# radiocosmology/cora

Hardware: AMD Instinct MI355X
Metric: sky-maps/sec (nside=1024, lmax=2048, 256 freq) (higher is better)
Workload: dtype f64

## Files before the change

cora_amd/csrc/fft_shapes.h:

```cpp
#pragma once
#include <cstddef>
#include <type_traits>
#include <utility>

namespace fft_shapes {

struct ring_shape {
    int len;
    int nch;
    int mc;
    int t;
    int ana_t;
    bool own;
    double us;
};
inline constexpr ring_shape RING_DIRECT[] = {
    {2048, 4, 4, 512, 512, false, 9.9},
    {4096, 2, 8, 512, 512, false, 12.7},
};
inline constexpr ring_shape RING_BLU[] = {
    {8192, 1, 16, 256, 0, true, 26.1},
    {6144, 1, 8, 512, 0, true, 20.5},
    {4096, 2, 4, 512, 512, false, 15.0},
    {3584, 2, 4, 512, 512, true, 14.3},
    {3072, 2, 4, 512, 512, true, 13.3},
    {2560, 2, 4, 512, 512, true, 12.4},
    {2048, 4, 2, 512, 512, false, 12.6},
    {1536, 4, 2, 512, 512, true, 10.6},
    {1024, 4, 2, 256, 256, false, 6.8},
};
constexpr bool has_analysis(const ring_shape &s) { return s.ana_t != 0; }
constexpr bool own_filter(const ring_shape &s) { return s.own; }

struct line_shape {
    int len;
    int nch;
    int t = 512;
    int t_c2r = 512;
    bool h2 = false;
    int inner_min = 0;
};
inline constexpr line_shape LINE_REAL[] = {
    {256, 16, 512, 256}, {512, 16}, {1024, 8}, {2048, 4}, {192, 16, 512, 256}, {384, 16}, {768, 8}, {1536, 4},
};
inline constexpr line_shape LINE_C2C[] = {
    {256, 16, 256, 256, false, 16}, {512, 16, 512, 512, false, 16}, {1024, 16, 512, 512, true, 16},
    {1024, 8, 512, 512, false, 8},  {384, 16, 512, 512, false, 16}, {768, 8, 512, 512, false, 8},
};
inline constexpr line_shape LINE_BLU[] = {
    {256, 16},  {320, 16},  {384, 16},  {512, 16},  {640, 8},  {768, 8},  {1024, 8},
    {1280, 4},  {1536, 4},  {2048, 4},  {2560, 2},  {3072, 2}, {3584, 2}, {4096, 2},
};
constexpr int LINE_BLU_FILTER_T = 256;

template <size_t N>
constexpr bool whole_loads(const line_shape (&rows)[N]) {
    for (const line_shape &s : rows)
        if ((s.nch * s.len) % s.t != 0 || (s.nch * s.len) % s.t_c2r != 0) return false;
    return true;
}
static_assert(whole_loads(LINE_REAL) && whole_loads(LINE_C2C) && whole_loads(LINE_BLU), "(NCH * N) % T == 0");

template <class S, size_t N>
constexpr const S *find(const S (&rows)[N], int len) {
    for (const S &s : rows)
        if (s.len == len) return &s;
    return nullptr;
}
constexpr int ring_own_length(int h, int P) {
    int best = 0;
    for (const ring_shape &s : RING_BLU)
        if (s.own && s.len >= 2 * h - 1 && s.len <= P && (best == 0 || s.len < best)) best = s.len;
    return best;
}

template <const auto &ROWS, size_t I>
struct row_c {
    static constexpr auto row = ROWS[I];
};
template <auto KEEP, class S>
constexpr bool kept(const S &s) {
    if constexpr (std::is_null_pointer_v<decltype(KEEP)>) return true;
    else return KEEP(s);
}
template <const auto &ROWS, auto KEEP, size_t... I, class Match, class Launch>
int dispatch_rows(std::index_sequence<I...>, Match match, Launch launch, bool *took) {
    int rc = 0;
    auto one = [&](auto shape) {
        if constexpr (kept<KEEP>(shape.row)) {
            if (!match(shape.row)) return false;
            rc = launch(shape);
            *took = rc == 0;
            return true;
        } else {
            return false;
        }
    };
    (void)(one(row_c<ROWS, I>{}) || ...);
    return rc;
}
template <const auto &ROWS, auto KEEP = nullptr, class Match, class Launch>
int dispatch(Match match, Launch launch, bool *took) {
    *took = false;
    return dispatch_rows<ROWS, KEEP>(std::make_index_sequence<sizeof(ROWS) / sizeof(ROWS[0])>{}, match, launch, took);
}

template <template <int> class SCH, const auto &ROWS, size_t... I>
constexpr bool scheduled(std::index_sequence<I...>) {
    return ((SCH<ROWS[I].len>::R0 * SCH<ROWS[I].len>::R1 * SCH<ROWS[I].len>::R2 == ROWS[I].len) && ...);
}
template <template <int> class SCH, const auto &ROWS>
// ... 6 lines not shown
```

cora_amd/csrc/sht_internal.h:

```cpp
#pragma once
#include "common.h"

#include <algorithm>
#include <cmath>
#include <type_traits>
#include <cstdlib>
#include <map>

struct corahip_sht_plan {
    int nside = 0, lmax = 0, L = 0, npair = 0, nring = 0;
    int cut_exp = 0;
    std::map<int, uint64_t> k4_macro_steps;
    std::map<std::pair<int, int>, std::pair<int2 *, int>> k4_items;
    std::vector<int32_t> h_lmin;
    long npix = 0, nalm = 0;
    std::vector<int64_t> h_start;
    std::vector<int32_t> h_nphi;
    std::vector<double> h_z, h_sth, h_phi0;
    double *d_z = nullptr, *d_sth = nullptr;
    int32_t *d_nphi = nullptr;
    int64_t *d_start = nullptr;
    double *d_phi0 = nullptr;
    double2 *d_coef = nullptr;
    int32_t *d_lstart = nullptr;
// ... 375 lines not shown
                    zv.x *= invP;
                    zv.y *= invP;
                    *reinterpret_cast<double2 *>(out + 2 * jj) = zv;
                }
            }
        }
    }
}
#ifndef K5_MC_BLU4
#define K5_MC_BLU4 2
#endif
#define K5_MC 4
#ifndef K5_STAMPS
#define K5_STAMPS 0
#endif
#if K5_STAMPS
__device__ unsigned long long g_k5_stamps[8];
#define K5STAMP(acc) { unsigned long long _t; asm volatile("s_memtime %0\n\ts_waitcnt lgkmcnt(0)" : "=s"(_t)::"memory"); acc += _t - k5_last; k5_last = _t; }
#else
#define K5STAMP(acc)
#endif
static inline int nnu_pad_of(int nnu) { return (nnu + 7) & ~7; }
#define K5_TAIL_PAD ((size_t)8 * 512 * 64)

int sht_legendre(corahip_ctx *ctx, const corahip_sht_plan *p, int ncols, const double *alm, double *inter);
int sht_k4_items(corahip_ctx *ctx, const corahip_sht_plan *p, int rt, int ncg, const int2 **items, int *nitems);
int sht_k4_segseed(corahip_ctx *ctx, const corahip_sht_plan *p, int rt, const double2 **segseed);
int sht_legendre_pol(corahip_ctx *ctx, corahip_sht_plan *p, int ncols, const double *alm, double *inter);
int sht_ringfft(corahip_ctx *ctx, const corahip_sht_plan *p, const double *inter, int nnu_chunk_pad, int nnu_valid,
                double *maps);
int sht_ringfft_ct(corahip_ctx *ctx, const corahip_sht_plan *p, const corahip_sht_plan::ring_class &c, const double *inter,
                   int G, int nnu, double *maps, int cu_limit, bool *took);
bool sht_ringfft_ticketed(const corahip_sht_plan::ring_class &c);
double sht_ringfft_item_weight(const corahip_sht_plan::ring_class &c);
#define K5_NTICKETS 8
int sht_k5_tickets(corahip_ctx *ctx, hipStream_t stream);
int sht_ctfilt_tables(corahip_ctx *ctx, corahip_sht_plan *p);
int sht_second_stream(corahip_ctx *ctx);
struct StreamRestore {
    corahip_ctx *c;
    hipStream_t s;
    bool forked = false;
    int fork() {
        const int rc = sht_second_stream(c);
        if (rc) return rc;
        HIP_TRY(hipEventRecord(c->ev_fork, s));
        HIP_TRY(hipStreamWaitEvent(c->stream2, c->ev_fork, 0));
        forked = true;
        return 0;
    }
    int join() {
        c->stream = s;
        HIP_TRY(hipEventRecord(c->ev_join, c->stream2));
        HIP_TRY(hipStreamWaitEvent(s, c->ev_join, 0));
        forked = false;
        return 0;
    }
    ~StreamRestore() {
        c->stream = s;
        if (forked && (hipEventRecord(c->ev_join, c->stream2) != hipSuccess || hipStreamWaitEvent(s, c->ev_join, 0) != hipSuccess))
            (void)hipStreamSynchronize(c->stream2);
    }
};
int sht_ringana_ct(corahip_ctx *ctx, const corahip_sht_plan *p, const corahip_sht_plan::ring_class &c, const double *maps, int nvalid,
                   int nnu_pad, const double *ring_w, int G, double *inter, bool *took);
int sht_ringana(corahip_ctx *ctx, const corahip_sht_plan *p, const double *maps, int nnu, int nnu_pad8,
                const double *ring_w, double *inter);
int sht_legendre_adj(corahip_ctx *ctx, const corahip_sht_plan *p, int ncols, const double *inter, double *part,
// ... 2 lines not shown
```

cora_amd/csrc/sht_ringfft.hip:

```cpp
#include "sht_internal.h"

template <int NCH, bool BLU>
__global__ void __launch_bounds__(K5_THREADS)
ringfft_kernel(const int32_t *__restrict__ ring_list, int nlist, int nside, int lmax, int G, int nnu, long npix,
               const int32_t *__restrict__ nphi_a, const int64_t *__restrict__ start_a,
               const double *__restrict__ phi0_a, const double *__restrict__ inter, double *__restrict__ maps,
               const double2 *__restrict__ tw_hbm, int pmax, const int32_t *__restrict__ blu_P,
               const int64_t *__restrict__ boff, const int64_t *__restrict__ foff,
               const double2 *__restrict__ chirp, const double2 *__restrict__ filt, int bstride,
               const int32_t *__restrict__ mcut) {
    constexpr int MC = BLU ? (NCH == 4 ? K5_MC_BLU4 : (K5_MC > 2 ? 2 : K5_MC)) : K5_MC;
    extern __shared__ __attribute__((aligned(16))) double2 sm[];
    const int tid = threadIdx.x, nt = blockDim.x;
    const int L = lmax + 1;
    const int ngrp = (nnu + NCH - 1) / NCH;
    const int nitems = nlist * ngrp;
    double *smd = reinterpret_cast<double *>(sm);
    const double2 *tw = tw_hbm;

    struct cell_t {
        double re[NCH], im[NCH];
    };
    cell_t pf0, pf1, pf2, pf3;
    auto cell_ptr = [&](int item) {
// ... 370 lines not shown
                *reinterpret_cast<double2 *>(cell + 4) = make_double2(im[0], im[1 % NCH]);
            } else {
                cell[0] = re[0];
                cell[4] = im[0];
            }
        }
    }
}
namespace {
struct ClassTimer {
    bool on;
    hipStream_t stream;
    hipEvent_t e0 = nullptr, e1 = nullptr;
    ClassTimer(bool on_, hipStream_t stream_) : on(on_), stream(stream_) {
        if (!on) return;
        (void)hipEventCreate(&e0);
        (void)hipEventCreate(&e1);
        (void)hipEventRecord(e0, stream);
    }
    void report(const char *kernel, const corahip_sht_plan::ring_class &c, int cus) {
        if (!on) return;
        float ms = 0.f;
        (void)hipEventRecord(e1, stream);
        (void)hipEventSynchronize(e1);
        (void)hipEventElapsedTime(&ms, e0, e1);
        fprintf(stderr, "%s class P=%d (length %d) nch=%d rings=%d: %.3f ms on %d CUs\n", kernel, c.blu ? c.len : 0, c.length(), c.nch,
                c.count, ms, cus);
        (void)hipEventDestroy(e0);
        (void)hipEventDestroy(e1);
    }
};
}

static int ringfft_launch_class(corahip_ctx *ctx, const corahip_sht_plan *p, const corahip_sht_plan::ring_class &c,
                                const double *inter, int G, int nnu_valid, double *maps, int cu_limit) {
    bool took = false;
    const int rct = sht_ringfft_ct(ctx, p, c, inter, G, nnu_valid, maps, cu_limit, &took);
    if (rct) return rct;
    if (took) return 0;
    const size_t shm = sizeof(double2) * (size_t)c.nch * c.bstride;
    const long nitems = (long)c.count * ((nnu_valid + c.nch - 1) / c.nch);
    const int per_cu = std::max<int>(1, (int)((160 * 1024) / std::max<size_t>(shm, 1)));
    const int k5_threads = c.threads ? c.threads : K5_THREADS;
    dim3 grid((unsigned)std::min<long>(nitems, (long)cu_limit * std::min(per_cu, k5_threads <= 128 ? 8 : 4)));
#define RINGFFT_LAUNCH(NCH, BLU)                                                                                     \
    HIP_TRY(hipFuncSetAttribute((const void *)ringfft_kernel<NCH, BLU>, hipFuncAttributeMaxDynamicSharedMemorySize,  \
                                160 * 1024));                                                                   \
    ringfft_kernel<NCH, BLU><<<grid, k5_threads, shm, ctx->stream>>>(c.d_list, c.count, p->nside, p->lmax, G, nnu_valid, p->npix,     \
                                                         p->d_nphi, p->d_start, p->d_phi0, inter, maps, p->d_tw, \
                                                         p->pmax, p->d_blu_P, p->d_blu_boff, p->d_blu_foff,      \
                                                         p->d_bchirp, p->d_bfilt, c.bstride, p->d_mcut)
    if (!c.blu) {
        if (c.nch == 4) { RINGFFT_LAUNCH(4, false); }
        else if (c.nch == 2) { RINGFFT_LAUNCH(2, false); }
        else { RINGFFT_LAUNCH(1, false); }
    } else {
        if (c.nch == 4) { RINGFFT_LAUNCH(4, true); }
        else if (c.nch == 2) { RINGFFT_LAUNCH(2, true); }
        else { RINGFFT_LAUNCH(1, true); }
    }
#undef RINGFFT_LAUNCH
    LAUNCH_CHECK();
    return 0;
}

static int k5_belt_wgs_switch() {
    const char *e = getenv("CORAHIP_K5_BELT_WGS");
    if (!e || !*e) return -1;
    return std::max(0, atoi(e));
}

int sht_ringfft(corahip_ctx *ctx, const corahip_sht_plan *p, const double *inter, int nnu_chunk_pad, int nnu_valid,
                       double *maps) {
    {
        StageTimer t(ctx, "ringfft");
        const int G = nnu_chunk_pad / 4;
        static const bool class_times = getenv("CORAHIP_K5_TIMES") != nullptr;
        const bool two = !class_times && !K5_STAMPS && p->classes.size() > 1;
        hipStream_t const main_stream = ctx->stream;
        StreamRestore restore{ctx, main_stream};
        const int ncu = ctx->num_cu;

        const corahip_sht_plan::ring_class *belt = nullptr;
        std::vector<std::pair<double, const corahip_sht_plan::ring_class *>> side;
        double B = 0.0, C = 0.0;
        for (const auto &c : p->classes) {
            const double cost = 1e-3 * sht_ringfft_item_weight(c) * (double)c.count * ((nnu_valid + c.nch - 1) / c.nch);
            if (!belt && sht_ringfft_ticketed(c)) {
                belt = &c;
                B = cost;
            } else {
                side.push_back({cost, &c});
                C += cost;
            }
        }
        if (belt) {
            const int rct = sht_k5_tickets(ctx, main_stream);
            if (rct) return rct;
        }
        const int sw = k5_belt_wgs_switch();
        int W = 0;
        if (two && belt && !side.empty() && sw != 0 && ncu >= 16 && ncu % 8 == 0) {
            if (sw > 0) {
                W = std::min(std::max(8 * ((sw + 4) / 8), 8), ncu - 8);
            } else if (B >= 0.2 * ncu && C >= 0.2 * ncu) {
                int gran = 8;
                for (const auto &sc : side) gran = std::max(gran, sc.second->nch == 2 ? 16 : (sc.second->nch == 1 ? 32 : 8));
                if (ncu % gran) gran = 8;
                const double share = C / (B + C) * ncu;
                int S = gran * (int)std::ceil(share / gran + 0.1);
                S = std::min(std::max(S, gran), ncu - 8);
                W = ncu - S;
            }
        }
        if (W > 0) {
            int rc = restore.fork();
            if (rc) return rc;
            if ((rc = ringfft_launch_class(ctx, p, *belt, inter, G, nnu_valid, maps, W))) return rc;
            ctx->stream = ctx->stream2;
            std::stable_sort(side.begin(), side.end(), [](const auto &a, const auto &b) { return a.first > b.first; });
            for (const auto &sc : side)
                if ((rc = ringfft_launch_class(ctx, p, *sc.second, inter, G, nnu_valid, maps, ncu - W))) return rc;
            if ((rc = ringfft_launch_class(ctx, p, *belt, inter, G, nnu_valid, maps, ncu - W))) return rc;
            return restore.join();
        }

        int rc = two ? restore.fork() : 0;
        if (rc) return rc;
        int launch_no = 0;
        for (const auto &c : p->classes) {
            if (two) ctx->stream = (launch_no++ & 1) ? ctx->stream2 : main_stream;
            ClassTimer timer(class_times, ctx->stream);
            const int cus = (class_times && sw > 0 && &c == belt) ? std::min(sw, ncu) : ncu;
            if ((rc = ringfft_launch_class(ctx, p, c, inter, G, nnu_valid, maps, cus))) return rc;
            timer.report("K5", c, cus);
#if K5_STAMPS
            {
                unsigned long long hs[8];
                HIP_TRY(hipStreamSynchronize(ctx->stream));
                HIP_TRY(hipMemcpyFromSymbol(hs, HIP_SYMBOL(g_k5_stamps), sizeof(hs)));
                fprintf(stderr, "K5 class P=%d nch=%d rings=%d: pre %llu zero %llu fold %llu z %llu fft %llu out %llu mid %llu dit %llu\n",
                        c.blu ? c.len : 0, c.nch, c.count, hs[0], hs[1], hs[2], hs[3], hs[4], hs[5], hs[6], hs[7]);
                unsigned long long z8[8] = {0};
                HIP_TRY(hipMemcpyToSymbol(HIP_SYMBOL(g_k5_stamps), z8, sizeof(z8)));
            }
#endif
        }
        if (two) return restore.join();
    }
    return 0;
}

int sht_ringana(corahip_ctx *ctx, const corahip_sht_plan *p, const double *maps, int nnu, int nnu_pad8,
                const double *ring_w, double *inter) {
    StageTimer t(ctx, "ringana");
    const int G = nnu_pad8 / 4;
// ... 35 lines not shown
```

cora_amd/csrc/sht_ringfft_ct.hip:

```cpp
#include "sht_internal.h"

#define CT_T 512
#ifndef CT_STAMPS
#define CT_STAMPS 0
#endif
#if CT_STAMPS
__device__ unsigned long long g_ct_stamps[12];
#define CTSTAMP(k) { unsigned long long _t; asm volatile("s_memtime %0\n\ts_waitcnt lgkmcnt(0)" : "=s"(_t)::"memory"); ct_acc[k] += _t - ct_last; ct_last = _t; }
#else
#define CTSTAMP(k)
#endif

#include "fft_ct.h"
#include "fft_shapes.h"
static_assert(fft_shapes::scheduled<Sch, fft_shapes::RING_DIRECT>() && fft_shapes::scheduled<Sch, fft_shapes::RING_BLU>(),
              "every ring shape has its three-pass schedule");

template <int NCH>
struct cell_ct {
    double re[NCH], im[NCH];
};
template <int NCH>
__device__ __forceinline__ static cell_ct<NCH> load_cell_ct(const double *cell, unsigned m) {
    cell_ct<NCH> c;
// ... 102 lines not shown
#pragma unroll
        for (int k = 0; k < MC; k++) {
            if (tid + k * T < Lr) fold_cell<PK, NCH, BS>(sm, tid + k * T, n, h, noalias, ph, pf[k]);
            ph = cmul(ph, phstep);
        }
        if (TAIL) {
            if (tid + MC * T < Lr) fold_cell<PK, NCH, BS>(sm, tid + MC * T, n, h, noalias, ph, pf[MC]);
            ph = cmul(ph, phstep);
        }
        for (int m = tid + (MC + (TAIL ? 1 : 0)) * T; m < Lr; m += T) {
            fold_cell<PK, NCH, BS>(sm, m, n, h, noalias, ph, load_cell_ct<NCH>(cell, m));
            ph = cmul(ph, phstep);
        }
    }
};

template <int NCH>
__device__ __forceinline__ static int ct_remap(int v, int nitems) {
    constexpr int SH = NCH == 2 ? 1 : (NCH == 1 ? 2 : 0);
    const bool on = SH > 0 && (nitems & ((8 << SH) - 1)) == 0 && (gridDim.x & ((8 << SH) - 1)) == 0;
    if (!on) return v;
    const int slot = v >> 3, xcd = v & 7;
    return (((slot >> SH) * 8 + xcd) << SH) + (slot & ((1 << SH) - 1));
}

template <int NCH>
__device__ __forceinline__ static int ct_remap_tk(int v, int nitems) {
    constexpr int SH = NCH == 2 ? 1 : (NCH == 1 ? 2 : 0);
    if (SH == 0 || (nitems & ((8 << SH) - 1)) != 0) return v;
    const int slot = v >> 3, xcd = v & 7;
    return (((slot >> SH) * 8 + xcd) << SH) + (slot & ((1 << SH) - 1));
}

template <int N, int NCH, int MC, int T>
__global__ void __launch_bounds__(T)
ringfft_direct_ct(const int32_t *__restrict__ ring_list, int nlist, int lmax, int G, int nnu, long npix,
                  const int64_t *__restrict__ start_a, const double *__restrict__ phi0_a,
                  const double *inter, double *maps, const int32_t *__restrict__ mcut, int *tickets) {
    constexpr int PK = K5_PK_DIRECT;
    constexpr int R0 = Sch<N>::R0, R1 = Sch<N>::R1, R2 = Sch<N>::R2;
    static_assert(R0 == 16 && R1 == 16, "digit map of the fused store assumes 16 x 16 x R2");
    constexpr int Q0 = N / R0;
    static_assert(Q0 % 128 == 0, "first-pass stride must be a multiple of the padding period");
    constexpr int BS = fpc(N) + 1 + K5_CH_SKEW;
    constexpr int n = 2 * N, h = N;
    extern __shared__ __attribute__((aligned(16))) double2 sm[];
    const int tid0 = threadIdx.x;
    const int L = lmax + 1;
    const int ngrp = (nnu + NCH - 1) / NCH;
    const int nitems = nlist * ngrp;

    constexpr bool PERX = NCH < 4;
    __shared__ int s_tk[2];
    int *ctr = tickets + (PERX ? (int)(blockIdx.x & 7) : 0);
    auto vitem_of = [&](int t) { return PERX ? 8 * t + (int)(blockIdx.x & 7) : t; };
    int tkn = 0;

    double2 wH, wA, wB;
    hermitian_twiddles<N, Q0, R1>(tid0, wH, wA, wB);
    auto cell_ptr = [&](int item) {
        const int ring = ring_list[item / ngrp];
        const int ch0 = (item % ngrp) * NCH;
        return inter + ((size_t)ring * G + (ch0 >> 2)) * L * 8 + (ch0 & 3);
    };
    FrontEnd<PK, NCH, BS, MC, true, T> fe;
    double2 phS, phstepS;
// ... 81 lines not shown
            constexpr int TOT = NCH * 256;
            constexpr int IT = (TOT + T - 1) / T;
            fe.touch();
            if (tid0 == 0) s_tk[1] = tkn;
#pragma unroll
            for (int it = 0; it < IT; it++) {
                const int idx = tid + it * T;
                if ((TOT % T) != 0 && idx >= TOT) break;
                const int ch = idx >> 8;
                int k0, k1;
                fused_digits<R0>(idx & 255, k0, k1);
                const double2 *p = sm + ch * BS + fused_slot<PK, R2>(k0, k1);
                double2 x[R2];
#pragma unroll
                for (int r = 0; r < R2; r++) x[r] = p[fpc(r)];
                DftR<R2, 1>::run(x);
                if (ch0 + ch < nnu) {
                    double *out = maps + (size_t)(ch0 + ch) * npix + start + 2 * (k0 + 16 * k1);
#pragma unroll
                    for (int r = 0; r < R2; r++) *reinterpret_cast<double2 *>(out + 512 * r) = x[r];
                }
            }
        }
        vitem = vnext;
    }
}

template <int P, int NCH, int MC, int T>
__global__ void __launch_bounds__(T)
ringfft_blu_ct(const int32_t *__restrict__ ring_list, int nlist, int nside, int lmax, int G, int nnu, long npix,
               const int32_t *__restrict__ nphi_a, const int64_t *__restrict__ start_a,
               const double *__restrict__ phi0_a, const double *inter, double *maps,
               const int64_t *__restrict__ boff, const int64_t *__restrict__ foff, const double2 *chirp,
               const double2 *filt, const int32_t *__restrict__ mcut, const double2 *foldph, const double2 *foldstep) {
    constexpr int PK = K5_PK_BLU;
    constexpr int R0 = Sch<P>::R0, R1 = Sch<P>::R1, R2 = Sch<P>::R2;
    constexpr int Q0 = P / R0;
    constexpr int BS = fpc(P) + K5_CH_SKEW;
    constexpr int HALF = (R0 / 2) * Q0;
    constexpr int U = (HALF / 2 + ((P & (P - 1)) ? 1 : 0) + T - 1) / T;
    extern __shared__ __attribute__((aligned(16))) double2 sm[];
    const int tid0 = threadIdx.x;
    const int L = lmax + 1;
    const int ngrp = (nnu + NCH - 1) / NCH;
    const int nitems = nlist * ngrp;
    const double invP = 1.0 / (double)P;

    double2 wA, wB;
    pass_twiddles<P, Q0, R1>(tid0, wA, wB);
    auto cell_ptr = [&](int item) {
        const int ring = ring_list[item / ngrp];
        const int ch0 = (item % ngrp) * NCH;
        return inter + ((size_t)ring * G + (ch0 >> 2)) * L * 8 + (ch0 & 3);
    };
    FrontEnd<PK, NCH, BS, MC, false, T, (U > 4 ? U : 4)> fe;
    double2 cbn[U];
    auto load_cbn = [&](int item, int t) {
        const int ring = ring_list[item / ngrp];
        const int ic = ring + 1 < nside ? ring + 1 : 4 * nside - (ring + 1);
        const double2 *b = chirp + boff[ic - 1];
        const int hh = nphi_a[ring] >> 1;
#pragma unroll
        for (int u = 0; u < U; u++) cbn[u] = b[min(t + u * T, hh - 1)];
    };
    int vitem = blockIdx.x;
    if (vitem < nitems) {
        fe.prefetch(cell_ptr(ct_remap<NCH>(vitem, nitems)), L, tid0);
        load_cbn(ct_remap<NCH>(vitem, nitems), tid0);
    }
    fe.touch();
#pragma unroll
    for (int u = 0; u < U; u++) asm volatile("" ::"v"(cbn[u].x), "v"(cbn[u].y));
#if CT_STAMPS
    unsigned long long ct_acc[12] = {0, 0, 0, 0, 0, 0, 0, 0, 0, 0, 0, 0}, ct_last;
    { unsigned long long _t; asm volatile("s_memtime %0\n\ts_waitcnt lgkmcnt(0)" : "=s"(_t)::"memory"); ct_last = _t; }
#endif
    for (; vitem < nitems; vitem += gridDim.x) {
        int tid = tid0;
        asm volatile("" : "+v"(tid));
        const int item = ct_remap<NCH>(vitem, nitems);
        const int ring = ring_list[item / ngrp];
        const int ch0 = (item % ngrp) * NCH;
        const int n = nphi_a[ring];
        const int h = n >> 1;
        const long start = start_a[ring];
        const int icap = ring + 1 < nside ? ring + 1 : 4 * nside - (ring + 1);
        const int Lr = mcut[ring];
        const double2 *bch = chirp + boff[icap - 1];
        constexpr int BPT = (P / R2 + T - 1) / T;
        const double2 *f = filt + foff[icap - 1] + (size_t)(tid % (P / R2)) * R2;
        constexpr bool FL_EARLY = !(R0 > 16 && T == 512);
        double2 fl[BPT][R2];
        if constexpr (FL_EARLY)
#pragma unroll
        for (int q = 0; q < BPT; q++)
#pragma unroll
            for (int r = 0; r < (R2 + 1) / 2; r++) fl[q][r] = f[(size_t)min(q * T, P / R2 - 1 - (int)(tid % (P / R2))) * R2 + r];
        const double2 fph0 = foldph[(size_t)(icap - 1) * 512 + tid];
        const double2 fphs = foldstep[(icap - 1) * 2 + (T == 512 ? 1 : 0)];
        double2 cb[U];
#pragma unroll
        for (int u = 0; u < U; u++) cb[u] = cbn[u];
        __syncthreads();
        CTSTAMP(0);
        fe.fold(sm, cell_ptr(item), Lr, n, fph0, fphs, tid);
        CTSTAMP(1);
        if constexpr (FL_EARLY)
#pragma unroll
        for (int q = 0; q < BPT; q++)
#pragma unroll
            for (int r = (R2 + 1) / 2; r < R2; r++) fl[q][r] = f[(size_t)min(q * T, P / R2 - 1 - (int)(tid % (P / R2))) * R2 + r];
        __syncthreads();
        CTSTAMP(2);
        static_assert(U <= decltype(fe)::KP, "the pre-pass takes w^k from the fold phases that are kept");
#pragma unroll
        for (int u = 0; u < U; u++) {
            const int k = tid + u * T;
            if (2 * k <= h) {
                const int k2 = h - k;
                const double2 wk = csqr(fe.phk[u]);
                const double2 iw = make_double2(-wk.y, wk.x);
                const double2 miwc = make_double2(-wk.y, -wk.x);
#pragma unroll
                for (int c = 0; c < NCH; c++) {
                    double2 *bc = sm + c * BS;
                    const double2 xa = bc[fpad(k)], xb = bc[fpad(k2)];
                    const double2 s1 = make_double2(xa.x + xb.x, xa.y - xb.y), d1 = make_double2(xa.x - xb.x, xa.y + xb.y);
                    const double2 s2 = make_double2(s1.x, -s1.y), d2 = make_double2(-d1.x, d1.y);
                    const double2 zk = cmul(cb[u], cadd(s1, cmul(iw, d1)));
                    const double2 zk2 = cmul(cb[u], cadd(s2, cmul(miwc, d2)));
                    bc[fpad(k)] = zk;
                    if (k > 0) {
                        if (k2 != k) bc[fpad(k2)] = zk2;
                    } else {
                        bc[fpad(h)] = make_double2(0.0, 0.0);
                    }
                }
            }
        }
        for (int j = h + 1 + tid; j < HALF; j += T)
#pragma unroll
            for (int c = 0; c < NCH; c++) sm[c * BS + fpad(j)] = make_double2(0.0, 0.0);
        const int nitem = ct_remap<NCH>(min(vitem + (int)gridDim.x, nitems - 1), nitems);
        fe.template prefetch<0>(cell_ptr(nitem), L, tid);
        __syncthreads();
        CTSTAMP(3);
        {
            constexpr int TOT = NCH * Q0;
            constexpr int IT = (TOT + T - 1) / T;
            const double2 w = cconj(wA);
#pragma unroll
            for (int it = 0; it < IT; it++) {
                const int idx = tid + it * T;
                if ((TOT % T) != 0 && idx >= TOT) break;
                const int ch = idx / Q0, j0 = idx & (Q0 - 1);
                double2 *p = sm + ch * BS + fpad(j0);
                double2 x[R0];
#pragma unroll
                for (int r = 0; r < R0 / 2; r++) x[r] = p[fpc(r * Q0)];
#pragma unroll
                for (int r = R0 / 2; r < R0; r++) x[r] = make_double2(0.0, 0.0);
                DftR<R0, -1>::run(x);
                tw_apply<R0>(x, w);
#pragma unroll
                for (int r = 0; r < R0; r++) p[fpc(r * Q0)] = x[r];
            }
        }
        fe.template prefetch<1>(cell_ptr(nitem), L, tid);
        load_cbn(nitem, tid);
        if constexpr (!FL_EARLY) {
#pragma unroll
            for (int r = 0; r < R2; r++) fl[0][r] = f[r];
        }
        __syncthreads();
        CTSTAMP(4);
        ct_pass<PK, P, NCH, BS, Q0, R1, -1, false, T>(sm, wB, tid);
// ... 14 lines not shown
                    for (int r = 0; r < R2; r++) x[r] = p[fpc(r)];
                    DftR<R2, -1>::run(x);
#pragma unroll
                    for (int r = 0; r < R2; r++) x[r] = cmul(x[r], fl[0][r]);
                    DftR<R2, 1>::run(x);
#pragma unroll
                    for (int r = 0; r < R2; r++) p[fpc(r)] = x[r];
                }
            } else {
#pragma unroll
                for (int ch = 0; ch < NCH; ch++)
#pragma unroll
                    for (int q = 0; q < BPT; q++) {
                        if ((NB % T) != 0 && tid + q * T >= NB) break;
                        double2 *p = sm + ch * BS + fpad((tid + q * T) * R2);
                        double2 x[R2];
#pragma unroll
                        for (int r = 0; r < R2; r++) x[r] = p[fpc(r)];
                        DftR<R2, -1>::run(x);
#pragma unroll
                        for (int r = 0; r < R2; r++) x[r] = cmul(x[r], fl[q][r]);
                        DftR<R2, 1>::run(x);
#pragma unroll
                        for (int r = 0; r < R2; r++) p[fpc(r)] = x[r];
                    }
            }
        }
        constexpr bool OB_EARLY = R0 <= 16;
        double2 ob[R0 / 2];
        if constexpr (OB_EARLY) blu_out_chirps<P>(ob, bch, tid & (Q0 - 1), h);
        __syncthreads();
        CTSTAMP(6);
        ct_pass<PK, P, NCH, BS, Q0, R1, 1, true, T>(sm, wB, tid);
        __syncthreads();
        CTSTAMP(7);
        {
            constexpr int TOT = NCH * Q0;
            constexpr int IT = (TOT + T - 1) / T;
#pragma unroll
            for (int it = 0; it < IT; it++) {
                const int idx = tid + it * T;
                if ((TOT % T) != 0 && idx >= TOT) break;
                const int ch = idx / Q0, j0 = idx & (Q0 - 1);
                const double2 *p = sm + ch * BS + fpad(j0);
                double2 x[R0];
#pragma unroll
                for (int r = 0; r < R0; r++) x[r] = p[fpc(r * Q0)];
                tw_apply<R0>(x, wA);
                DftR<R0, 1>::run(x);
                if (ch0 + ch < nnu) {
                    double *out = maps + (size_t)(ch0 + ch) * npix + start;
#pragma unroll
                    for (int r = 0; r < R0 / 2; r++) {
                        const int jj = j0 + r * Q0;
                        if (jj < h) {
                            double2 zv = cmul(x[r], OB_EARLY ? ob[r] : bch[jj]);
                            zv.x *= invP;
                            zv.y *= invP;
                            *reinterpret_cast<double2 *>(out + 2 * jj) = zv;
                        }
                    }
                }
            }
        }
        CTSTAMP(8);
    }
#if CT_STAMPS
    if ((tid0 & 63) == 0)
        for (int k = 0; k < 9; k++) atomicAdd(&g_ct_stamps[k], ct_acc[k]);
#endif
}

template <int N, int NCH, int T>
__global__ void __launch_bounds__(T)
ringana_direct_ct(const int32_t *__restrict__ ring_list, int nlist, int lmax, int G, int nnu, int nvalid, long npix,
                  const int64_t *__restrict__ start_a, const double *__restrict__ phi0_a, const double *maps, double *inter,
                  const int32_t *__restrict__ mcut, const double *__restrict__ ring_w, int nring) {
    constexpr int PK = K5_PK_DIRECT;
    constexpr int R0 = Sch<N>::R0, R1 = Sch<N>::R1, R2 = Sch<N>::R2;
    static_assert(R0 == 16 && R1 == 16, "digit map of the fused load assumes 16 x 16 x R2");
    constexpr int Q0 = N / R0;
    static_assert(Q0 % 128 == 0, "first-pass stride must be a multiple of the padding period");
    constexpr int BS = fpc(N) + 1 + K5_CH_SKEW;
    constexpr int TOT0 = NCH * 256, IT0 = (TOT0 + T - 1) / T;
    static_assert(TOT0 % T == 0, "every thread loads whole butterflies");
    constexpr int MO = N / T;
    extern __shared__ __attribute__((aligned(16))) double2 sm[];
    const int tid0 = threadIdx.x;
    const int L = lmax + 1;
    const int ngrp = (nnu + NCH - 1) / NCH;
    const int nitems = nlist * ngrp;

    double2 wA, wB;
    double2 wS, wSstep;
    double2 phS, phSstep;
    pass_twiddles<N, Q0, R1>(tid0, wA, wB);
    {
        double s, c;
// ... 74 lines not shown
#pragma unroll
            for (int u = 0; u < MO; u++) {
                const int m = tid + u * T;
                if (m < Lr) emit(m, w, ph);
                w = cmul(w, wSstep);
                ph = cmul(ph, phstep);
            }
            if (tid == 0 && N < Lr) emit(N, make_double2(-1.0, 0.0), shifted ? make_double2(0.0, -1.0) : make_double2(1.0, 0.0));
        }
    }
}

template <int N, int NCH, int MC, int T>
static int launch_direct(corahip_ctx *ctx, hipStream_t stream, const corahip_sht_plan *p,
                         const corahip_sht_plan::ring_class &c, const double *inter, int G, int nnu, double *maps, int cu_limit) {
    constexpr int PK = K5_PK_DIRECT;
    constexpr int BS = fpc(N) + 1 + K5_CH_SKEW;
    const long nitems = (long)c.count * ((nnu + NCH - 1) / NCH);
    const auto [shm, grid] = ct_launch_geom(NCH, BS, 0, 0, nitems, cu_limit);
    if (!ctx->k5_tickets) {
        corahip_set_error("ring FFT: the ticket counters of the context are missing");
        return CORAHIP_ESTATE;
    }
    static_assert(sizeof(double2) * (size_t)NCH * BS + 64 <= 160 * 1024, "channel buffers + ticket words fit the LDS");
    HIP_TRY(hipFuncSetAttribute((const void *)ringfft_direct_ct<N, NCH, MC, T>, hipFuncAttributeMaxDynamicSharedMemorySize,
                                (int)shm));
    ringfft_direct_ct<N, NCH, MC, T><<<grid, T, shm, stream>>>(c.d_list, c.count, p->lmax, G, nnu, p->npix, p->d_start,
                                                               p->d_phi0, inter, maps, p->d_mcut, ctx->k5_tickets);
    LAUNCH_CHECK();
    return 0;
}
template <int P, int NCH, int MC, int T>
static int launch_blu(corahip_ctx *ctx, hipStream_t stream, const corahip_sht_plan *p,
                      const corahip_sht_plan::ring_class &c, const double *inter, int G, int nnu, double *maps, int cu_limit) {
    const int64_t *d_foff = c.ct_own ? p->d_ctfilt_off : p->d_blu_foff;
    const double2 *d_filt = c.ct_own ? p->d_ctfilt : p->d_bfilt;
    constexpr int PK = K5_PK_BLU;
    constexpr int BS = fpc(P) + K5_CH_SKEW;
    static_assert(sizeof(double2) * (size_t)NCH * BS <= 160 * 1024, "channel buffers fit the LDS");
    const long nitems = (long)c.count * ((nnu + NCH - 1) / NCH);
    const auto [shm, grid] = ct_launch_geom(NCH, BS, 0, 0, nitems, cu_limit);
    HIP_TRY(hipFuncSetAttribute((const void *)ringfft_blu_ct<P, NCH, MC, T>, hipFuncAttributeMaxDynamicSharedMemorySize,
                                160 * 1024));
    ringfft_blu_ct<P, NCH, MC, T><<<grid, T, shm, stream>>>(c.d_list, c.count, p->nside, p->lmax, G, nnu, p->npix, p->d_nphi,
                                                            p->d_start, p->d_phi0, inter, maps, p->d_blu_boff,
                                                            d_foff, p->d_bchirp, d_filt, p->d_mcut, p->d_foldph, p->d_foldstep);
    LAUNCH_CHECK();
#if CT_STAMPS
    {
        unsigned long long hs[12], z[12] = {0};
        HIP_TRY(hipStreamSynchronize(stream));
        HIP_TRY(hipMemcpyFromSymbol(hs, HIP_SYMBOL(g_ct_stamps), sizeof(hs)));
        const double per = 1.0 / ((double)nitems * (T / 64));
        fprintf(stderr, "K5ct P=%d nch=%d items=%ld: cycles/item  top %.0f fold %.0f pf+bar %.0f pre %.0f F1 %.0f F2 %.0f mid %.0f I2 %.0f I3 %.0f\n",
                P, NCH, nitems, hs[0] * per, hs[1] * per, hs[2] * per, hs[3] * per, hs[4] * per, hs[5] * per, hs[6] * per,
                hs[7] * per, hs[8] * per);
        HIP_TRY(hipMemcpyToSymbol(HIP_SYMBOL(g_ct_stamps), z, sizeof(z)));
    }
#endif
    return 0;
}

int sht_ringfft_ct(corahip_ctx *ctx, const corahip_sht_plan *p, const corahip_sht_plan::ring_class &c, const double *inter,
                   int G, int nnu, double *maps, int cu_limit, bool *took) {
    const auto len_is = [&](const fft_shapes::ring_shape &s) { return s.len == c.ct_len; };
    if (!c.blu)
        return fft_shapes::dispatch<fft_shapes::RING_DIRECT>(len_is, [&](auto shape) {
            return launch_direct<shape.row.len, shape.row.nch, shape.row.mc, shape.row.t>(ctx, ctx->stream, p, c, inter, G, nnu, maps, cu_limit);
        }, took);
    return fft_shapes::dispatch<fft_shapes::RING_BLU>(len_is, [&](auto shape) {
        return launch_blu<shape.row.len, shape.row.nch, shape.row.mc, shape.row.t>(ctx, ctx->stream, p, c, inter, G, nnu, maps, cu_limit);
    }, took);
}

template <int P, int NCH, int T>
__global__ void __launch_bounds__(T)
ringana_blu_ct(const int32_t *__restrict__ ring_list, int nlist, int nside, int lmax, int G, int nnu, int nvalid, long npix,
               const int32_t *__restrict__ nphi_a, const int64_t *__restrict__ start_a, const double *maps, double *inter,
               const int64_t *__restrict__ boff, const int64_t *__restrict__ foff, const double2 *chirp, const double2 *filt,
               const int32_t *__restrict__ mcut, const double2 *foldph, const double2 *foldstep, const double *__restrict__ ring_w) {
    constexpr int PK = K5_PK_BLU;
    constexpr int R0 = Sch<P>::R0, R1 = Sch<P>::R1, R2 = Sch<P>::R2;
    static_assert(R0 <= 16, "the lengths above 4096 keep the generic kernel");
    constexpr int Q0 = P / R0;
    constexpr int BS = fpc(P) + K5_CH_SKEW;
    constexpr int HALF = (R0 / 2) * Q0;
    constexpr int U = (HALF + T - 1) / T;
    constexpr int NB = P / R2;
    static_assert(NB <= T, "one middle-stage butterfly per thread and channel group");
    extern __shared__ __attribute__((aligned(16))) double2 sm[];
    const int tid0 = threadIdx.x;
    const int L = lmax + 1;
    const int ngrp = (nnu + NCH - 1) / NCH;
    const int nitems = nlist * ngrp;
    const int nring = 4 * nside - 1;
    const double invP = 1.0 / (double)P;

    double2 wA, wB;
    pass_twiddles<P, Q0, R1>(tid0, wA, wB);
    double2 pf[NCH][U];
    double2 cbn[U];
    auto prefetch = [&](int item, int t) {
        const int ring = ring_list[item / ngrp];
        const int ch0 = (item % ngrp) * NCH;
// ... 163 lines not shown
}
template <int P, int NCH, int T>
static int launch_ana_blu(corahip_ctx *ctx, hipStream_t stream, const corahip_sht_plan *p, const corahip_sht_plan::ring_class &c,
                          const double *maps, int nvalid, int nnu_pad, const double *ring_w, int G, double *inter) {
    constexpr int PK = K5_PK_BLU;
    constexpr int BS = fpc(P) + K5_CH_SKEW;
    static_assert(sizeof(double2) * (size_t)NCH * BS <= 160 * 1024, "channel buffers fit the LDS");
    const long nitems = (long)c.count * ((nnu_pad + NCH - 1) / NCH);
    const auto [shm, grid] = ct_launch_geom(NCH, BS, 0, 0, nitems, ctx->num_cu);
    HIP_TRY(hipFuncSetAttribute((const void *)ringana_blu_ct<P, NCH, T>, hipFuncAttributeMaxDynamicSharedMemorySize, 160 * 1024));
    ringana_blu_ct<P, NCH, T><<<grid, T, shm, stream>>>(c.d_list, c.count, p->nside, p->lmax, G, nnu_pad, nvalid, p->npix, p->d_nphi,
                                                        p->d_start, maps, inter, p->d_blu_boff, c.ct_own ? p->d_ctfilt_off : p->d_blu_foff,
                                                        p->d_bchirp, c.ct_own ? p->d_ctfilt : p->d_bfilt, p->d_mcut, p->d_foldph,
                                                        p->d_foldstep, ring_w);
    LAUNCH_CHECK();
    return 0;
}
int sht_ringana_ct(corahip_ctx *ctx, const corahip_sht_plan *p, const corahip_sht_plan::ring_class &c, const double *maps, int nvalid,
                   int nnu_pad, const double *ring_w, int G, double *inter, bool *took) {
    *took = false;
    if (nvalid < 1) return 0;
    const auto len_is = [&](const fft_shapes::ring_shape &s) { return s.len == c.ct_len; };
    if (c.blu)
        return fft_shapes::dispatch<fft_shapes::RING_BLU, fft_shapes::has_analysis>(len_is, [&](auto shape) {
            return launch_ana_blu<shape.row.len, shape.row.nch, shape.row.ana_t>(ctx, ctx->stream, p, c, maps, nvalid, nnu_pad, ring_w, G, inter);
        }, took);
    if (p->lmax > c.len) return 0;
    return fft_shapes::dispatch<fft_shapes::RING_DIRECT, fft_shapes::has_analysis>(len_is, [&](auto shape) {
        return launch_ana_direct<shape.row.len, shape.row.nch, shape.row.ana_t>(ctx, ctx->stream, p, c, maps, nvalid, nnu_pad, ring_w, G, inter);
    }, took);
}

bool sht_ringfft_ticketed(const corahip_sht_plan::ring_class &c) { return !c.blu && c.ct_len != 0; }

double sht_ringfft_item_weight(const corahip_sht_plan::ring_class &c) {
    if (const fft_shapes::ring_shape *s = c.blu ? fft_shapes::find(fft_shapes::RING_BLU, c.ct_len) : fft_shapes::find(fft_shapes::RING_DIRECT, c.ct_len))
        return s->us;
    if (!c.blu) return 13.0;
    return c.len > 4096 ? 26.1 * c.len / 8192 : 5.7;
}

int sht_k5_tickets(corahip_ctx *ctx, hipStream_t stream) {
    if (!ctx->k5_tickets) HIP_TRY(hipMalloc((void **)&ctx->k5_tickets, sizeof(int) * K5_NTICKETS));
    HIP_TRY(hipMemsetAsync(ctx->k5_tickets, 0, sizeof(int) * K5_NTICKETS, stream));
    return 0;
}

int sht_second_stream(corahip_ctx *ctx) {
    if (!ctx->stream2) {
        HIP_TRY(hipStreamCreateWithFlags(&ctx->stream2, hipStreamNonBlocking));
        HIP_TRY(hipEventCreateWithFlags(&ctx->ev_fork, hipEventDisableTiming));
        HIP_TRY(hipEventCreateWithFlags(&ctx->ev_join, hipEventDisableTiming));
    }
    return 0;
}

template <int P>
__global__ void __launch_bounds__(CT_T)
blu3_filter_kernel(int nside, const int32_t *__restrict__ p3_of, const int64_t *__restrict__ boff, const int64_t *__restrict__ foff3,
                   const double2 *__restrict__ chirp, double2 *__restrict__ filt3) {
    constexpr int PK = K5_PK_BLU;
    constexpr int BS = fpc(P) + K5_CH_SKEW;
    extern __shared__ __attribute__((aligned(16))) double2 sm[];
    const int i = blockIdx.x + 1;
    if (p3_of[i - 1] != P) return;
    const int tid = threadIdx.x;
// ... 37 lines not shown
```

Measured before the change: 3294.

## Hand out Bluestein ring FFT items with atomic tickets and relaunch on both streams

The Bluestein ring-FFT kernel now gets its work items from per-class atomic ticket counters, with per-XCD counters when there are fewer than four channels, in place of a fixed grid stride. Each Bluestein class is then launched a second time on the main stream after the split, so blocks on both stream partitions drain the same pool. The ticket buffer grows to sixteen counter sets, and the side-partition granularity and rounding logic are changed. The aim is to balance load across the two-stream CU split and remove tail idle time, at the cost of atomic traffic and extra launches. An environment switch to force the generic kernel and adjusted cost weights are also added.

```diff
diff --git a/cora_amd/csrc/fft_shapes.h b/cora_amd/csrc/fft_shapes.h
--- a/cora_amd/csrc/fft_shapes.h
+++ b/cora_amd/csrc/fft_shapes.h
@@ -20,14 +20,14 @@
 };
 inline constexpr ring_shape RING_BLU[] = {
     {8192, 1, 16, 256, 0, true, 26.1},
-    {6144, 1, 8, 512, 0, true, 20.5},
+    {6144, 1, 8, 512, 0, true, 19.8},
     {4096, 2, 4, 512, 512, false, 15.0},
     {3584, 2, 4, 512, 512, true, 14.3},
     {3072, 2, 4, 512, 512, true, 13.3},
     {2560, 2, 4, 512, 512, true, 12.4},
     {2048, 4, 2, 512, 512, false, 12.6},
     {1536, 4, 2, 512, 512, true, 10.6},
-    {1024, 4, 2, 256, 256, false, 6.8},
+    {1024, 4, 2, 256, 256, false, 6.4},
 };
 constexpr bool has_analysis(const ring_shape &s) { return s.ana_t != 0; }
 constexpr bool own_filter(const ring_shape &s) { return s.own; }
@@ -77,6 +77,7 @@
 template <const auto &ROWS, size_t I>
 struct row_c {
     static constexpr auto row = ROWS[I];
+    static constexpr size_t index = I;
 };
 template <auto KEEP, class S>
 constexpr bool kept(const S &s) {
diff --git a/cora_amd/csrc/sht_internal.h b/cora_amd/csrc/sht_internal.h
--- a/cora_amd/csrc/sht_internal.h
+++ b/cora_amd/csrc/sht_internal.h
@@ -431,8 +431,10 @@
 int sht_ringfft_ct(corahip_ctx *ctx, const corahip_sht_plan *p, const corahip_sht_plan::ring_class &c, const double *inter,
                    int G, int nnu, double *maps, int cu_limit, bool *took);
 bool sht_ringfft_ticketed(const corahip_sht_plan::ring_class &c);
+bool sht_ringfft_cap_ticketed(const corahip_sht_plan::ring_class &c);
 double sht_ringfft_item_weight(const corahip_sht_plan::ring_class &c);
-#define K5_NTICKETS 8
+#define K5_TICKET_SETS 16
+#define K5_NTICKETS (8 * K5_TICKET_SETS)
 int sht_k5_tickets(corahip_ctx *ctx, hipStream_t stream);
 int sht_ctfilt_tables(corahip_ctx *ctx, corahip_sht_plan *p);
 int sht_second_stream(corahip_ctx *ctx);
diff --git a/cora_amd/csrc/sht_ringfft.hip b/cora_amd/csrc/sht_ringfft.hip
--- a/cora_amd/csrc/sht_ringfft.hip
+++ b/cora_amd/csrc/sht_ringfft.hip
@@ -426,11 +426,18 @@
 };
 }
 
+static bool k5_generic_switch() {
+    const char *e = getenv("CORAHIP_K5_GENERIC");
+    return e && *e && atoi(e) != 0;
+}
+
 static int ringfft_launch_class(corahip_ctx *ctx, const corahip_sht_plan *p, const corahip_sht_plan::ring_class &c,
                                 const double *inter, int G, int nnu_valid, double *maps, int cu_limit) {
     bool took = false;
-    const int rct = sht_ringfft_ct(ctx, p, c, inter, G, nnu_valid, maps, cu_limit, &took);
-    if (rct) return rct;
+    if (!k5_generic_switch()) {
+        const int rct = sht_ringfft_ct(ctx, p, c, inter, G, nnu_valid, maps, cu_limit, &took);
+        if (rct) return rct;
+    }
     if (took) return 0;
     const size_t shm = sizeof(double2) * (size_t)c.nch * c.bstride;
     const long nitems = (long)c.count * ((nnu_valid + c.nch - 1) / c.nch);
@@ -478,9 +485,11 @@
         const corahip_sht_plan::ring_class *belt = nullptr;
         std::vector<std::pair<double, const corahip_sht_plan::ring_class *>> side;
         double B = 0.0, C = 0.0;
+        bool tickets = false;
         for (const auto &c : p->classes) {
             const double cost = 1e-3 * sht_ringfft_item_weight(c) * (double)c.count * ((nnu_valid + c.nch - 1) / c.nch);
-            if (!belt && sht_ringfft_ticketed(c)) {
+            tickets = tickets || sht_ringfft_ticketed(c) || sht_ringfft_cap_ticketed(c);
+            if (!belt && sht_ringfft_ticketed(c) && !k5_generic_switch()) {
                 belt = &c;
                 B = cost;
             } else {
@@ -488,7 +497,7 @@
                 C += cost;
             }
         }
-        if (belt) {
+        if (tickets) {
             const int rct = sht_k5_tickets(ctx, main_stream);
             if (rct) return rct;
         }
@@ -499,10 +508,12 @@
                 W = std::min(std::max(8 * ((sw + 4) / 8), 8), ncu - 8);
             } else if (B >= 0.2 * ncu && C >= 0.2 * ncu) {
                 int gran = 8;
-                for (const auto &sc : side) gran = std::max(gran, sc.second->nch == 2 ? 16 : (sc.second->nch == 1 ? 32 : 8));
+                for (const auto &sc : side)
+                    if (!sht_ringfft_cap_ticketed(*sc.second) && sc.first >= 0.2 * ncu)
+                        gran = std::max(gran, sc.second->nch == 2 ? 16 : (sc.second->nch == 1 ? 32 : 8));
                 if (ncu % gran) gran = 8;
                 const double share = C / (B + C) * ncu;
-                int S = gran * (int)std::ceil(share / gran + 0.1);
+                int S = gran == 8 ? 8 * (int)std::lround(share / 8) : gran * (int)std::ceil(share / gran + 0.1);
                 S = std::min(std::max(S, gran), ncu - 8);
                 W = ncu - S;
             }
@@ -510,12 +521,16 @@
         if (W > 0) {
             int rc = restore.fork();
             if (rc) return rc;
+            std::stable_sort(side.begin(), side.end(), [](const auto &a, const auto &b) { return a.first > b.first; });
             if ((rc = ringfft_launch_class(ctx, p, *belt, inter, G, nnu_valid, maps, W))) return rc;
             ctx->stream = ctx->stream2;
-            std::stable_sort(side.begin(), side.end(), [](const auto &a, const auto &b) { return a.first > b.first; });
             for (const auto &sc : side)
                 if ((rc = ringfft_launch_class(ctx, p, *sc.second, inter, G, nnu_valid, maps, ncu - W))) return rc;
             if ((rc = ringfft_launch_class(ctx, p, *belt, inter, G, nnu_valid, maps, ncu - W))) return rc;
+            ctx->stream = main_stream;
+            for (const auto &sc : side)
+                if (sht_ringfft_cap_ticketed(*sc.second))
+                    if ((rc = ringfft_launch_class(ctx, p, *sc.second, inter, G, nnu_valid, maps, W))) return rc;
             return restore.join();
         }
 
diff --git a/cora_amd/csrc/sht_ringfft_ct.hip b/cora_amd/csrc/sht_ringfft_ct.hip
--- a/cora_amd/csrc/sht_ringfft_ct.hip
+++ b/cora_amd/csrc/sht_ringfft_ct.hip
@@ -158,6 +158,9 @@
     return (((slot >> SH) * 8 + xcd) << SH) + (slot & ((1 << SH) - 1));
 }
 
+constexpr bool blu_ticketed(int P, int T) { return true; }
+static_assert(1 + sizeof(fft_shapes::RING_BLU) / sizeof(fft_shapes::RING_BLU[0]) <= K5_TICKET_SETS, "one counter set per ticketed class");
+
 template <int N, int NCH, int MC, int T>
 __global__ void __launch_bounds__(T)
 ringfft_direct_ct(const int32_t *__restrict__ ring_list, int nlist, int lmax, int G, int nnu, long npix,
@@ -305,7 +308,8 @@
                const int32_t *__restrict__ nphi_a, const int64_t *__restrict__ start_a,
                const double *__restrict__ phi0_a, const double *inter, double *maps,
                const int64_t *__restrict__ boff, const int64_t *__restrict__ foff, const double2 *chirp,
-               const double2 *filt, const int32_t *__restrict__ mcut, const double2 *foldph, const double2 *foldstep) {
+               const double2 *filt, const int32_t *__restrict__ mcut, const double2 *foldph, const double2 *foldstep,
+               int *tickets) {
     constexpr int PK = K5_PK_BLU;
     constexpr int R0 = Sch<P>::R0, R1 = Sch<P>::R1, R2 = Sch<P>::R2;
     constexpr int Q0 = P / R0;
@@ -336,10 +340,26 @@
 #pragma unroll
         for (int u = 0; u < U; u++) cbn[u] = b[min(t + u * T, hh - 1)];
     };
+    constexpr bool TK = blu_ticketed(P, T);
+    constexpr bool PERX = NCH < 4;
+    __shared__ int s_tk[2];
+    int *ctr = tickets + (PERX ? (int)(blockIdx.x & 7) : 0);
+    auto vitem_of = [&](int t) { return PERX ? 8 * t + (int)(blockIdx.x & 7) : t; };
+    auto remap = [&](int v) { return TK ? ct_remap_tk<NCH>(v, nitems) : ct_remap<NCH>(v, nitems); };
+    int tkn = 0;
     int vitem = blockIdx.x;
+    if constexpr (TK) {
+        if (tid0 == 0) {
+            tkn = atomicAdd(ctr, 2);
+            s_tk[0] = tkn;
+            s_tk[1] = tkn + 1;
+        }
+        __syncthreads();
+        vitem = vitem_of(__builtin_amdgcn_readfirstlane(s_tk[0]));
+    }
     if (vitem < nitems) {
-        fe.prefetch(cell_ptr(ct_remap<NCH>(vitem, nitems)), L, tid0);
-        load_cbn(ct_remap<NCH>(vitem, nitems), tid0);
+        fe.prefetch(cell_ptr(remap(vitem)), L, tid0);
+        load_cbn(remap(vitem), tid0);
     }
     fe.touch();
 #pragma unroll
@@ -348,10 +368,10 @@
     unsigned long long ct_acc[12] = {0, 0, 0, 0, 0, 0, 0, 0, 0, 0, 0, 0}, ct_last;
     { unsigned long long _t; asm volatile("s_memtime %0\n\ts_waitcnt lgkmcnt(0)" : "=s"(_t)::"memory"); ct_last = _t; }
 #endif
-    for (; vitem < nitems; vitem += gridDim.x) {
+    while (vitem < nitems) {
         int tid = tid0;
         asm volatile("" : "+v"(tid));
-        const int item = ct_remap<NCH>(vitem, nitems);
+        const int item = remap(vitem);
         const int ring = ring_list[item / ngrp];
         const int ch0 = (item % ngrp) * NCH;
         const int n = nphi_a[ring];
@@ -414,7 +434,14 @@
         for (int j = h + 1 + tid; j < HALF; j += T)
 #pragma unroll
             for (int c = 0; c < NCH; c++) sm[c * BS + fpad(j)] = make_double2(0.0, 0.0);
-        const int nitem = ct_remap<NCH>(min(vitem + (int)gridDim.x, nitems - 1), nitems);
+        int vnext, nitem;
+        if constexpr (TK) {
+            vnext = vitem_of(__builtin_amdgcn_readfirstlane(s_tk[1]));
+            nitem = remap(vnext < nitems ? vnext : vitem);
+        } else {
+            vnext = vitem + (int)gridDim.x;
+            nitem = remap(min(vnext, nitems - 1));
+        }
         fe.template prefetch<0>(cell_ptr(nitem), L, tid);
         __syncthreads();
         CTSTAMP(3);
@@ -495,11 +522,21 @@
         __syncthreads();
         CTSTAMP(6);
         ct_pass<PK, P, NCH, BS, Q0, R1, 1, true, T>(sm, wB, tid);
+        if constexpr (TK) {
+            if (tid0 == 0) {
+                auto c = (__attribute__((address_space(1))) int *)ctr;
+                asm volatile("" : "+v"(c));
+                tkn = __hip_atomic_fetch_add(c, 1, __ATOMIC_RELAXED, __HIP_MEMORY_SCOPE_AGENT);
+            }
+        }
         __syncthreads();
         CTSTAMP(7);
         {
             constexpr int TOT = NCH * Q0;
             constexpr int IT = (TOT + T - 1) / T;
+            if constexpr (TK && !OB_EARLY) {
+                if (tid0 == 0) s_tk[1] = tkn;
+            }
 #pragma unroll
             for (int it = 0; it < IT; it++) {
                 const int idx = tid + it * T;
@@ -511,6 +548,12 @@
                 for (int r = 0; r < R0; r++) x[r] = p[fpc(r * Q0)];
                 tw_apply<R0>(x, wA);
                 DftR<R0, 1>::run(x);
+                if constexpr (TK && OB_EARLY) {
+                    if (it == 0) {
+                        asm volatile("" : "+v"(x[0].x), "+v"(x[R0 / 2 - 1].y));
+                        if (tid0 == 0) s_tk[1] = tkn;
+                    }
+                }
                 if (ch0 + ch < nnu) {
                     double *out = maps + (size_t)(ch0 + ch) * npix + start;
 #pragma unroll
@@ -527,6 +570,7 @@
             }
         }
         CTSTAMP(8);
+        vitem = vnext;
     }
 #if CT_STAMPS
     if ((tid0 & 63) == 0)
@@ -667,19 +711,25 @@
 }
 template <int P, int NCH, int MC, int T>
 static int launch_blu(corahip_ctx *ctx, hipStream_t stream, const corahip_sht_plan *p,
-                      const corahip_sht_plan::ring_class &c, const double *inter, int G, int nnu, double *maps, int cu_limit) {
+                      const corahip_sht_plan::ring_class &c, const double *inter, int G, int nnu, double *maps, int cu_limit,
+                      int ticket_set) {
     const int64_t *d_foff = c.ct_own ? p->d_ctfilt_off : p->d_blu_foff;
     const double2 *d_filt = c.ct_own ? p->d_ctfilt : p->d_bfilt;
     constexpr int PK = K5_PK_BLU;
     constexpr int BS = fpc(P) + K5_CH_SKEW;
-    static_assert(sizeof(double2) * (size_t)NCH * BS <= 160 * 1024, "channel buffers fit the LDS");
+    static_assert(sizeof(double2) * (size_t)NCH * BS + 64 <= 160 * 1024, "channel buffers + ticket words fit the LDS");
     const long nitems = (long)c.count * ((nnu + NCH - 1) / NCH);
     const auto [shm, grid] = ct_launch_geom(NCH, BS, 0, 0, nitems, cu_limit);
+    if (blu_ticketed(P, T) && !ctx->k5_tickets) {
+        corahip_set_error("ring FFT: the ticket counters of the context are missing");
+        return CORAHIP_ESTATE;
+    }
     HIP_TRY(hipFuncSetAttribute((const void *)ringfft_blu_ct<P, NCH, MC, T>, hipFuncAttributeMaxDynamicSharedMemorySize,
-                                160 * 1024));
+                                (int)shm));
     ringfft_blu_ct<P, NCH, MC, T><<<grid, T, shm, stream>>>(c.d_list, c.count, p->nside, p->lmax, G, nnu, p->npix, p->d_nphi,
                                                             p->d_start, p->d_phi0, inter, maps, p->d_blu_boff,
-                                                            d_foff, p->d_bchirp, d_filt, p->d_mcut, p->d_foldph, p->d_foldstep);
+                                                            d_foff, p->d_bchirp, d_filt, p->d_mcut, p->d_foldph, p->d_foldstep,
+                                                            ctx->k5_tickets ? ctx->k5_tickets + 8 * ticket_set : nullptr);
     LAUNCH_CHECK();
 #if CT_STAMPS
     {
@@ -704,7 +754,8 @@
             return launch_direct<shape.row.len, shape.row.nch, shape.row.mc, shape.row.t>(ctx, ctx->stream, p, c, inter, G, nnu, maps, cu_limit);
         }, took);
     return fft_shapes::dispatch<fft_shapes::RING_BLU>(len_is, [&](auto shape) {
-        return launch_blu<shape.row.len, shape.row.nch, shape.row.mc, shape.row.t>(ctx, ctx->stream, p, c, inter, G, nnu, maps, cu_limit);
+        return launch_blu<shape.row.len, shape.row.nch, shape.row.mc, shape.row.t>(ctx, ctx->stream, p, c, inter, G, nnu, maps, cu_limit,
+                                                                                   1 + (int)shape.index);
     }, took);
 }
 
@@ -934,6 +985,11 @@
 }
 
 bool sht_ringfft_ticketed(const corahip_sht_plan::ring_class &c) { return !c.blu && c.ct_len != 0; }
+bool sht_ringfft_cap_ticketed(const corahip_sht_plan::ring_class &c) {
+    if (!c.blu) return false;
+    const fft_shapes::ring_shape *s = fft_shapes::find(fft_shapes::RING_BLU, c.ct_len);
+    return s && blu_ticketed(s->len, s->t);
+}
 
 double sht_ringfft_item_weight(const corahip_sht_plan::ring_class &c) {
     if (const fft_shapes::ring_shape *s = c.blu ? fft_shapes::find(fft_shapes::RING_BLU, c.ct_len) : fft_shapes::find(fft_shapes::RING_DIRECT, c.ct_len))
```

Result: no change. 3316, median of 6 (+0.7%).
